# MohaMehrzad/aiOS

Measured on AMD Instinct MI355X. Metric: decode tokens/sec Mistral-7B Q4_K (aggregate over GPUs), higher is better.
Workload: dtype q8_1-act/Q4_K_M; 1 GPU; model=Mistral-7B-Instruct-v0.2 Q4_K_M (architecture: d4096 L32 H32/8 ff14336 V32000), global_batch=1, seq_len=2012, parallelism=dp1, weights=Q4_K_M, per_gpu_batch=1, hipgraph=True

## Files before the change

aios_amd/csrc/bindings.cpp:

```cpp
#include <pybind11/numpy.h>
#include <pybind11/pybind11.h>
#include <pybind11/stl.h>

#include <cstring>

#include "comm.h"
#include "rccl_comm.h"
#include "engine.h"
#include "grammar.h"
#include "ops.h"

namespace py = pybind11;
using namespace aios;

namespace aios {
double bench_launch_chain(int n_kernels, int blocks, int use_graph, int reps);
double bench_stream_read(size_t bytes, int nbuf, int wg_per_cu, int u, int threads, int reps);
double bench_stream_read_part(size_t bytes, int nbuf, int mode, int threads, int reps);
}

namespace {

hipStream_t S(uintptr_t s) { return reinterpret_cast<hipStream_t>(s); }

// ... 427 lines not shown
          a.ts = (unsigned long long*)ts;
          a.block_table = (const int*)block_table; a.bt_rows = bt_rows;
          a.q = (const float*)q; a.k_cache = (const bf16_t*)k; a.v_cache = (const bf16_t*)v;
          a.seq_len = (const int*)seq_len; a.slot = (const int*)slot;
          a.B = B; a.n_heads = H; a.n_kv_heads = Hkv; a.head_dim = hd; a.max_ctx = max_ctx; a.n_chunks = n_chunks;
          a.scale = scale; a.o_part = (float*)opart; a.ml = (float*)ml; a.out = (float*)out;
          a.counters = (int*)counters;
          launch_attn_decode(a, S(st));
        },
        py::arg("q"), py::arg("k"), py::arg("v"), py::arg("seq_len"), py::arg("slot"), py::arg("B"), py::arg("H"),
        py::arg("Hkv"), py::arg("hd"), py::arg("max_ctx"), py::arg("n_chunks"), py::arg("scale"), py::arg("opart"),
        py::arg("ml"), py::arg("out"), py::arg("counters"), py::arg("st"), py::arg("split") = 0,
        py::arg("block_table") = 0, py::arg("bt_rows") = 0, py::arg("ts") = 0, py::arg("kv_fp8") = 0,
        py::arg("k_scale") = 1.f, py::arg("v_scale") = 1.f);
  m.def("attn_decode_split", &attn_decode_split);
  m.def("device_cu_count", [](int dev) {
    int n = 0;
    HIP_CHECK(hipDeviceGetAttribute(&n, hipDeviceAttributeMultiprocessorCount, dev));
    return n;
  }, py::arg("device") = 0);
  m.def("device_pci_bus_id", [](int dev) {
    char buf[64] = {0};
    HIP_CHECK(hipDeviceGetPCIBusId(buf, (int)sizeof(buf), dev));
    return std::string(buf);
  });
  m.def("rmsnorm", [](uintptr_t x, int ldx, uintptr_t w, uintptr_t y, int ldy, int rows, int n, float eps, uintptr_t st) {
    launch_rmsnorm((const float*)x, ldx, (const float*)w, (float*)y, ldy, rows, n, eps, S(st));
  });
  m.def("rmsnorm_bf16", [](uintptr_t x, int ldx, uintptr_t w, uintptr_t y, int ldy, int rows, int n, float eps, uintptr_t st) {
    launch_rmsnorm_bf16((const float*)x, ldx, (const float*)w, (bf16_t*)y, ldy, rows, n, eps, S(st));
// ... 181 lines not shown
```

aios_amd/csrc/engine.hip:

```cpp
#include "engine.h"
#include <hip/hip_ext.h>

#include <set>
#include "comm.h"
#include <cstdlib>
#include <map>

#include <algorithm>
#include <cstring>
#include <cmath>
#include <regex>
#include <sstream>

#include <rocprofiler-sdk-roctx/roctx.h>

namespace aios {

static bool trace_enabled() {
  static const int on = [] {
    const char* e = std::getenv("AIOS_TRACE");
    return e && std::atoi(e) == 0 ? 0 : 1;
  }();
  return on != 0;
}
// ... 42 lines not shown
  if (!cfg_.cu_mask.empty()) {
    int n = 0, dev_cus = 0;
    for (uint32_t w : cfg_.cu_mask) n += __builtin_popcount(w);
    HIP_CHECK(hipDeviceGetAttribute(&dev_cus, hipDeviceAttributeMultiprocessorCount, cfg_.device));
    if (n <= 0) throw std::runtime_error("cu_mask selects no CU");
    HIP_CHECK(hipExtStreamCreateWithCUMask(&stream_, (uint32_t)cfg_.cu_mask.size(), cfg_.cu_mask.data()));
    cus_ = std::min(n, dev_cus);
  } else if (cfg_.stream_priority != 0) {
    int least = 0, greatest = 0;
    HIP_CHECK(hipDeviceGetStreamPriorityRange(&least, &greatest));
    const int pr = std::max(greatest, std::min(least, cfg_.stream_priority));
    HIP_CHECK(hipStreamCreateWithPriority(&stream_, hipStreamNonBlocking, pr));
  } else {
    HIP_CHECK(hipStreamCreateWithFlags(&stream_, hipStreamNonBlocking));
  }

  layers_.resize(cfg_.n_layers);
  if (cfg_.max_batch < 1 || cfg_.max_batch > 64) throw std::runtime_error("max_batch must be 1..64");
  if (cfg_.max_slots < cfg_.max_batch) cfg_.max_slots = cfg_.max_batch;
  if (cfg_.tp_size <= 1 || cfg_.tie_embeddings) cfg_.vocab_parallel = 0;
  if (cfg_.vocab_parallel && cfg_.vocab_size % cfg_.tp_size)
    throw std::runtime_error("vocab_parallel: vocab_size not divisible by tp_size");
}

Engine::~Engine() {
  try {
    stage_release();
  } catch (...) {
  }
  for (auto& kv : graphs_) hipGraphExecDestroy(kv.second);
// ... 1847 lines not shown
```

aios_amd/csrc/gemv.h:

```cpp
#pragma once
#include "common.h"
#include "qweight.h"

namespace aios {

constexpr int GEMV_MAX_SEGS = 3;

enum GemvEpilogue : int {
  EPI_STORE = 0,
  EPI_RESID = 1,
  EPI_SWIGLU = 2,
  EPI_QKV = 3,
  EPI_TP_RESID = 4,
};

struct ArDevCtx;

struct GemvArgs {
  QWeight seg[GEMV_MAX_SEGS];
  int seg_row0[GEMV_MAX_SEGS];
  int nseg;
  int N, K, B;
  int row_base;
  int kt_max;
// ... 22 lines not shown
  const int* pos;
  const int* slot;
  bf16_t* k_cache;
  const int* block_table;
  bf16_t* v_cache;
  int kv_fp8;
  float kv_inv_k, kv_inv_v;
  const int* step_kv;
  const float2* step_rope;
  const ArDevCtx* tp;
  int grid_cap;
  int dry;
};

void launch_gemv(const GemvArgs& a, hipStream_t st);
bool gemv_engine_fits(const GemvArgs& a);
bool gemv_bf16_engine_fits(const GemvArgs& a);
bool launch_gemv_tp_fused(const GemvArgs& a, hipStream_t st);

}
```

aios_amd/csrc/kernels/gemv_cu.h:

```cpp
#pragma once

constexpr int CU_WAVES = 16;
constexpr int CU_THREADS = CU_WAVES * 64;

struct CuPlan {
  int g0;
  int np0;
  int racc_n;
};

template <int CTRL>
__device__ __forceinline__ float cu_dpp(float v) {
  return __int_as_float(__builtin_amdgcn_mov_dpp(__float_as_int(v), CTRL, 0xF, 0xF, false));
}
__device__ __forceinline__ float cu_wave_sum(float v) {
  v += cu_dpp<0xB1>(v);
  v += cu_dpp<0x4E>(v);
  v += cu_dpp<0x141>(v);
  v += cu_dpp<0x140>(v);
  {
    const auto r = __builtin_amdgcn_permlane16_swap(__float_as_uint(v), __float_as_uint(v), false, false);
    v = __uint_as_float(r[0]) + __uint_as_float(r[1]);
  }
  {
// ... 193 lines not shown
  };
  cu_dispatch<DMAX>(min(DMAX, j1 - j0), [&](auto NC) { chunk(NC, std::true_type{}, j0); });
  for (int jb = j0 + DMAX; jb < j1; jb += DMAX)
    cu_dispatch<DMAX>(min(DMAX, j1 - jb), [&](auto NC) { chunk(NC, std::false_type{}, jb); });
  CU_STAMP(4);
}

template <int QT0, int QT1, int D>
__global__ void __launch_bounds__(CU_THREADS) gemv_cu_b1(GemvArgs a, CuPlan pl) {
  static_assert(same_xlayout<QT0, QT1>, "mixed segments must share the activation layout");
  extern __shared__ __attribute__((aligned(16))) float smem[];
  constexpr bool MIXED = QT0 != QT1;
  constexpr int W = QFmt<QT0>::W, R = QFmt<QT0>::RUNS;
  const int nch = a.K / W;
  const int nit = (nch + 63) >> 6;
  const int npairs = a.N >> 1;
  const int lane = threadIdx.x & 63, wave = threadIdx.x >> 6;
  unsigned long long ts[8] = {0, 0, 0, 0, 0, 0, 0, 0};
  CU_STAMP(0);
  auto flush_ts = [&]() {
    if (a.dbg_ts && lane == 0 && (wave == 0 || wave == CU_WAVES - 1))
      for (int i = 0; i < 8; ++i) a.dbg_ts[((size_t)blockIdx.x * 2 + (wave != 0)) * 8 + i] = ts[i];
  };

  const int g = blockIdx.x;
  const bool fmt1 = MIXED && g >= pl.g0;
  int pb, pe;
  if (!fmt1) {
    const int np = MIXED ? pl.np0 : npairs, G = MIXED ? pl.g0 : (int)gridDim.x;
    pb = (int)((long)g * np / G);
    pe = (int)((long)(g + 1) * np / G);
  } else {
    const int np = npairs - pl.np0, G = (int)gridDim.x - pl.g0, gg = g - pl.g0;
    pb = pl.np0 + (int)((long)gg * np / G);
    pe = pl.np0 + (int)((long)(gg + 1) * np / G);
  }
  if (pb >= pe) return;
  const int r0 = 2 * pb, nrows = 2 * (pe - pb);
  const int items = nrows * nit;
  const int ipw = (items + CU_WAVES - 1) / CU_WAVES;
  const int j0 = __builtin_amdgcn_readfirstlane(min(items, wave * ipw));
  const int j1 = __builtin_amdgcn_readfirstlane(min(items, j0 + ipw));

  float* red = smem;
  float* rowacc = smem + 64;
  const int racc_n = pl.racc_n;
  float2* ms = (float2*)(rowacc + racc_n);
  int8_t* xq = (int8_t*)(ms + (size_t)nch * R);
  for (int i = threadIdx.x; i < nrows; i += CU_THREADS) rowacc[i] = 0.f;

  float2 rope = make_float2(1.f, 0.f);
  if (!fmt1) cu_body<QT0, QT0, D>(a, r0, j0, j1, nit, nch, red, rowacc, ms, xq, rope, ts);
  else cu_body<QT1, QT0, D>(a, r0, j0, j1, nit, nch, red, rowacc, ms, xq, rope, ts);
  __syncthreads();
// ... 35 lines not shown
      cu_qkv_epilogue(a, grow, v0, v1, t, pos0, kv_blk0);
    } else {
      gemv_epilogue1(a, grow, v0, v1);
    }
  }
  CU_STAMP(6);
  flush_ts();
}

template <int QT0, int QT1>
inline size_t cu_lds_bytes(const GemvArgs& a, int racc_n) {
  constexpr int W = QFmt<QT0>::W, R = QFmt<QT0>::RUNS;
  return (64 + (size_t)racc_n) * 4 + (size_t)(a.K / W) * R * 8 + (size_t)a.K + 16;
}

inline int cu_fmt_bytes_per_256(int qt) {
  switch (qt) {
    case QT_Q4_K: return 144;
    case QT_Q5_K: return 176;
    case QT_Q6_K: return 210;
    case QT_Q4_0: return 144;
    case QT_Q8_0: return 272;
  }
  return 256;
}

template <int QT0, int QT1>
bool launch_gemv_cu(const GemvArgs& a, hipStream_t st) {
  if constexpr (!same_xlayout<QT0, QT1>) {
    return false;
  } else {
    static const int env = [] {
      const char* e = std::getenv("AIOS_GEMV_CU");
      return e ? std::atoi(e) : 0;
    }();
    const int mode = a.kernel_sel == 2 ? 8 : (a.kernel_sel == 0 ? env : 0);
    if (!mode || a.B != 1 || a.tune_dbg) return false;
    const int npairs = a.N / 2;
    const int cus = device_cu_count();
    const int G = std::min(a.tune_grid > 0 ? a.tune_grid : cus, npairs);
    auto rup = [](int n, int g) { return (n + g - 1) / g; };
    CuPlan pl{G, npairs, (2 * rup(npairs, G) + 3) & ~3};
    if (QT0 != QT1 && a.nseg > 1) {
      const int np0 = a.seg_row0[a.nseg - 1] / 2;
      const double b0 = (double)np0 * cu_fmt_bytes_per_256(QT0), b1 = (double)(npairs - np0) * cu_fmt_bytes_per_256(QT1);
      int g0 = (int)(G * b0 / (b0 + b1) + 0.5);
      g0 = std::max(1, std::min(G - 1, g0));
      if (G < 2 || np0 < 1 || np0 >= npairs) return false;
      const int most = std::max(rup(np0, g0), rup(npairs - np0, G - g0));
      pl = CuPlan{g0, np0, (2 * most + 3) & ~3};
    }
    size_t lds = cu_lds_bytes<QT0, QT1>(a, pl.racc_n);
    if (lds > 160 * 1024) return false;
    lds = std::max(lds, (size_t)(81 * 1024));
    if (mode <= 4)
      hipLaunchKernelGGL((gemv_cu_b1<QT0, QT1, 4>), dim3(G), dim3(CU_THREADS), lds, st, a, pl);
    else
      hipLaunchKernelGGL((gemv_cu_b1<QT0, QT1, 8>), dim3(G), dim3(CU_THREADS), lds, st, a, pl);
    return true;
  }
}
```

aios_amd/csrc/kernels/gemv_dispatch.hip:

```cpp
#include <stdexcept>
#include <string>

#include "../gemv.h"

namespace aios {
void gemv_q4k_q4k(const GemvArgs&, hipStream_t);
void gemv_q4k_q6k(const GemvArgs&, hipStream_t);
void gemv_q6k_q6k(const GemvArgs&, hipStream_t);
void gemv_q5k_q5k(const GemvArgs&, hipStream_t);
void gemv_q5k_q6k(const GemvArgs&, hipStream_t);
void gemv_q4_0(const GemvArgs&, hipStream_t);
void gemv_q8_0(const GemvArgs&, hipStream_t);
void gemv_f16(const GemvArgs&, hipStream_t);
void gemv_bf16(const GemvArgs&, hipStream_t);

bool gemv_q4k_q4k_engine_fits(const GemvArgs&);
bool gemv_q4k_q6k_engine_fits(const GemvArgs&);
bool gemv_q6k_q6k_engine_fits(const GemvArgs&);
bool gemv_q5k_q5k_engine_fits(const GemvArgs&);
bool gemv_q5k_q6k_engine_fits(const GemvArgs&);
bool gemv_q4_0_engine_fits(const GemvArgs&);
bool gemv_q8_0_engine_fits(const GemvArgs&);

bool gemv_engine_fits(const GemvArgs& a) {
// ... 72 lines not shown
```

aios_amd/csrc/kernels/gemv_impl.h:

```cpp
#pragma once
#include <algorithm>

#include "../comm.h"
#include "../common.h"
#include "../gemv.h"
#include "../qweight.h"

namespace aios {

__device__ __forceinline__ QWeight seg_at(const GemvArgs& a, int s) {
  QWeight w;
  w.qtype = s == 0 ? a.seg[0].qtype : (s == 1 ? a.seg[1].qtype : a.seg[2].qtype);
  w.rows = s == 0 ? a.seg[0].rows : (s == 1 ? a.seg[1].rows : a.seg[2].rows);
  w.cols = s == 0 ? a.seg[0].cols : (s == 1 ? a.seg[1].cols : a.seg[2].cols);
  w.pad_ = 0;
  w.p0 = s == 0 ? a.seg[0].p0 : (s == 1 ? a.seg[1].p0 : a.seg[2].p0);
  w.p1 = s == 0 ? a.seg[0].p1 : (s == 1 ? a.seg[1].p1 : a.seg[2].p1);
  w.p2 = s == 0 ? a.seg[0].p2 : (s == 1 ? a.seg[1].p2 : a.seg[2].p2);
  w.p3 = s == 0 ? a.seg[0].p3 : (s == 1 ? a.seg[1].p3 : a.seg[2].p3);
  return w;
}
__device__ __forceinline__ int seg_row0_at(const GemvArgs& a, int s) {
  return s == 0 ? a.seg_row0[0] : (s == 1 ? a.seg_row0[1] : a.seg_row0[2]);
}
// ... 539 lines not shown
```

aios_amd/csrc/kernels/gemv_lds.h:

```cpp
#pragma once

constexpr int LG_NG = 14;
constexpr int LG_NL = 2;
constexpr int LG_THREADS = (LG_NG + LG_NL) * 64;
constexpr int LG_DBG_RING = 0x10000;
#ifndef LG_B0
#define LG_B0 0
#endif

template <int QT>
struct LgPlanes;
template <>
struct LgPlanes<QT_Q4_K> {
  static constexpr int n = 2;
  static constexpr int bpg[4] = {1024, 128, 0, 0};
  static constexpr int dsz[4] = {16, 16, 0, 0};
};
template <>
struct LgPlanes<QT_Q5_K> {
  static constexpr int n = 3;
  static constexpr int bpg[4] = {1024, 128, 256, 0};
  static constexpr int dsz[4] = {16, 16, 16, 0};
};
template <>
// ... 36 lines not shown
}

__device__ __forceinline__ void lg_barrier() {
  asm volatile("" ::: "memory");
  __builtin_amdgcn_s_barrier();
  asm volatile("" ::: "memory");
}

template <int N>
__device__ __forceinline__ void lg_vmcnt() {
  static_assert(N >= 0 && N <= 63, "vmcnt immediate");
  asm volatile("s_waitcnt vmcnt(%0)" ::"n"(N) : "memory");
}

template <int QT>
__device__ __forceinline__ void lg_dma_slot(const GemvArgs& a, uint8_t* dst, int s, int lw, int r0, int nit,
                                            int ngroups) {
  using L = LgLayout<QT>;
  using P = LgPlanes<QT>;
  constexpr int NGS = L::NGS;
  const int lane = threadIdx.x & 63;
  const int g0 = r0 * nit + s * NGS;
  const int glast = r0 * nit + ngroups - 1;
  const int G1 = a.nseg > 1 ? a.seg_row0[1] * nit : 0x7fffffff;
  const int G2 = a.nseg > 2 ? a.seg_row0[2] * nit : 0x7fffffff;
  const int gend = g0 + NGS - 1;
  const int sg0 = g0 >= G2 ? 2 : (g0 >= G1 ? 1 : 0);
  const int Gs = sg0 == 0 ? 0 : (sg0 == 1 ? G1 : G2);
  const int Gn = sg0 == 0 ? G1 : (sg0 == 1 ? G2 : 0x7fffffff);
  const bool fast = gend <= glast && gend < Gn;
  int issued = 0;
  int idx = 0;
  static_for<4>([&](auto pc) {
    constexpr int p = decltype(pc)::value;
    if constexpr (p < P::n) {
      constexpr int S = P::dsz[p], BPG = P::bpg[p];
      constexpr int NI = L::ninst(p);
      const uint8_t* pb0 = sgpr_ptr(lg_plane_ptr(a.seg[0], p));
      const uint8_t* pb1 = sgpr_ptr(lg_plane_ptr(a.seg[1], p));
      const uint8_t* pb2 = sgpr_ptr(lg_plane_ptr(a.seg[2], p));
      if (fast) {
        const __amdgpu_buffer_rsrc_t rs = mk_rsrc(sg0 == 0 ? pb0 : (sg0 == 1 ? pb1 : pb2));
        const int soff0 = (g0 - Gs) * BPG;
#pragma unroll
        for (int i = 0; i < NI; ++i) {
          if ((idx + i) % LG_NL != lw) continue;
          auto* ldst = (__attribute__((address_space(3))) void*)(dst + L::off(p) + i * 64 * S);
          if constexpr (S == 16) __builtin_amdgcn_raw_ptr_buffer_load_lds(rs, ldst, 16, lane * 16, soff0 + i * 1024, 0, 2);
          else __builtin_amdgcn_raw_ptr_buffer_load_lds(rs, ldst, 4, lane * 4, soff0 + i * 256, 0, 2 );
          ++issued;
        }
      } else {
        const uint64_t b0 = (uint64_t)pb0;
        const uint64_t b1 = (uint64_t)pb1 - (uint64_t)(a.nseg > 1 ? G1 : 0) * BPG;
        const uint64_t b2 = (uint64_t)pb2 - (uint64_t)(a.nseg > 2 ? G2 : 0) * BPG;
#pragma unroll
        for (int i = 0; i < NI; ++i) {
          if ((idx + i) % LG_NL != lw) continue;
          const int b = i * 64 * S + lane * S;
          int g = g0 + b / BPG;
          const int o = b & (BPG - 1);
          g = min(g, glast);
          const uint64_t base = g >= G2 ? b2 : (g >= G1 ? b1 : b0);
          const uint8_t* src = (const uint8_t*)(base + (uint64_t)g * BPG + o);
          auto* ldst = (__attribute__((address_space(3))) void*)(dst + L::off(p) + i * 64 * S);
          if constexpr (S == 16) __builtin_amdgcn_global_load_lds((const void*)src, ldst, 16, 0, 2 );
          else __builtin_amdgcn_global_load_lds((const void*)src, ldst, 4, 0, 2 );
          ++issued;
        }
      }
      idx += NI;
    }
  });
  if (issued < L::per_loader) {
    const int g = min(g0, glast);
    const uint64_t b0 = (uint64_t)sgpr_ptr(a.seg[0].p0);
    const uint64_t b1 = (uint64_t)sgpr_ptr(a.seg[1].p0) - (uint64_t)(a.nseg > 1 ? G1 : 0) * 1024;
    const uint64_t b2 = (uint64_t)sgpr_ptr(a.seg[2].p0) - (uint64_t)(a.nseg > 2 ? G2 : 0) * 1024;
    const uint64_t base = g >= G2 ? b2 : (g >= G1 ? b1 : b0);
    const uint8_t* src = (const uint8_t*)(base + (uint64_t)g * 1024 + lane * 16);
    for (; issued < L::per_loader; ++issued)
      __builtin_amdgcn_global_load_lds((const void*)src, (__attribute__((address_space(3))) void*)dst, 16, 0, 2);
  }
}

template <int QT>
__device__ __forceinline__ void lg_read(const uint8_t* slot, int k, int lane, RawChunk& r) {
  using L = LgLayout<QT>;
  const uint8_t* A = slot + L::off(0) + k * 1024;
  r.a = *(const uint4*)(A + lane * 16);
  if constexpr (QT == QT_Q4_K || QT == QT_Q5_K) {
    r.b = *(const uint4*)(slot + L::off(1) + k * 128 + (lane >> 3) * 16);
    if constexpr (QT == QT_Q5_K) r.c = *(const uint4*)(slot + L::off(2) + k * 256 + (lane >> 3) * 32 + 16 * (lane & 1));
  } else if constexpr (QT == QT_Q6_K) {
    const uint2 h = *(const uint2*)(slot + L::off(1) + k * 512 + lane * 8);
    r.b.x = h.x;
    r.b.y = h.y;
    r.c.x = *(const uint16_t*)(slot + L::off(2) + k * 128 + lane * 2);
// ... 113 lines not shown
      if (!valid) m = make_float2(0.f, 0.f);
      acc[b] += sc[rr] * m.x * (float)is[rr] - of[rr] * m.y;
    }
  }
}

template <int QT0, int QT1, int B = 1, int RSUB = 0>
__global__ void __launch_bounds__(LG_THREADS) gemv_lds_b1(GemvArgs a, CuPlan pl) {
  static_assert(same_xlayout<QT0, QT1>, "mixed segments must share the activation layout");
  kernarg_warm<sizeof(GemvArgs) + sizeof(CuPlan)>();
  extern __shared__ __attribute__((aligned(16))) float smem[];
  constexpr bool MIXED = QT0 != QT1;
  constexpr int W = QFmt<QT0>::W, R = QFmt<QT0>::RUNS;
  const int nch = a.K / W;
  const int nit = nch >> 6;
  const int npairs = a.N >> 1;
  const int lane = threadIdx.x & 63;
  const int wave = __builtin_amdgcn_readfirstlane(threadIdx.x >> 6);
  const bool loader = wave >= LG_NG;
  unsigned long long ts[8] = {0, 0, 0, 0, 0, 0, 0, 0};
  CU_STAMP(0);

  const int g = blockIdx.x;
  const bool fmt1 = MIXED && g >= pl.g0;
  int pb, pe;
  if (!fmt1) {
    const int np = MIXED ? pl.np0 : npairs, G = MIXED ? pl.g0 : (int)gridDim.x;
    pb = (int)((long)g * np / G);
    pe = (int)((long)(g + 1) * np / G);
  } else {
    const int np = npairs - pl.np0, G = (int)gridDim.x - pl.g0, gg = g - pl.g0;
    pb = pl.np0 + (int)((long)gg * np / G);
    pe = pl.np0 + (int)((long)(gg + 1) * np / G);
  }
  if (pb >= pe) return;
  const int r0 = 2 * pb, nrows = 2 * (pe - pb);
  const int ngroups = nrows * nit;

  float* red = smem;
  float* rowacc = smem + 64;
  float2* ms = (float2*)(rowacc + B * pl.racc_n);
  int8_t* xq = (int8_t*)(ms + (size_t)B * nch * R);
  const int ring_off = (int)(((const uint8_t*)(xq + (size_t)B * a.K) - (const uint8_t*)smem + 255) & ~255);
  uint8_t* ring = (uint8_t*)smem + ring_off;
  for (int i = threadIdx.x; i < B * pl.racc_n; i += LG_THREADS) rowacc[i] = 0.f;
  if (threadIdx.x < 64) red[threadIdx.x] = 0.f;
  asm volatile("s_waitcnt lgkmcnt(0)" ::: "memory");

  auto loader_path = [&](auto tag) __attribute__((always_inline)) {
    constexpr int QT = decltype(tag)::value;
    using L = LgLayout<QT, RSUB>;
    constexpr int PL = L::per_loader;
    constexpr int LG_R = L::R;
    const int T = (ngroups + L::NGS - 1) / L::NGS;
    const int lw = wave - LG_NG;
    if (LG_B0) lg_barrier();
    const int npro = min(T, LG_R - 1);
    for (int s = 0; s < npro; ++s) lg_dma_slot<QT>(a, ring + (size_t)s * L::slot_bytes, s, lw, r0, nit, ngroups);
    if (npro == LG_R - 1) lg_vmcnt<(LG_R - 2) * PL>();
    else lg_vmcnt<0>();
    lg_barrier();
    for (int t = 0; t < T; ++t) {
      if (t + LG_R - 1 < T) {
        lg_dma_slot<QT>(a, ring + (size_t)((t + LG_R - 1) % LG_R) * L::slot_bytes, t + LG_R - 1, lw, r0, nit,
                        ngroups);
        lg_vmcnt<(LG_R - 2) * PL>();
      } else {
        lg_vmcnt<0>();
      }
      lg_barrier();
    }
    lg_barrier();
  };
  auto consumer_path = [&](auto tag, float2& rope, int& pos0, int& kv_blk0) __attribute__((always_inline)) {
    constexpr int QT = decltype(tag)::value;
    using L = LgLayout<QT, RSUB>;
    constexpr int LG_R = L::R;
    constexpr int GPW = L::GPW;
    const int T = (ngroups + L::NGS - 1) / L::NGS;
    constexpr int NPF = 2;
    StagePre<NPF> pf{};
    q8_stage_prefetch(a, pf, threadIdx.x, LG_NG * 64);
    if (LG_B0) lg_barrier();
    CU_STAMP(1);
    q8_stage<QT0, B, NPF>(a, xq, ms, red, pf, threadIdx.x, LG_NG * 64);
    if (B == 1 && a.epi == EPI_QKV && wave == 0) {
      pos0 = a.pos[0];
      kv_blk0 = kv_block(a.block_table, a.max_ctx / KV_BLOCK, a.slot ? a.slot[0] : 0, pos0);
      if (a.rope_cs) {
        int part, head, lrr;
        qkv_part(a, a.row_base + r0 + 2 * lane, part, head, lrr);
        rope = a.rope_cs[(size_t)pos0 * (a.head_dim >> 1) + (part < 2 ? (lrr >> 1) : 0)];
      }
    }
// ... 203 lines not shown
      }
      lg_barrier();
    }
    CU_STAMP(4);
    asm volatile("s_waitcnt lgkmcnt(0)" ::: "memory");
    lg_barrier();
    CU_STAMP(5);
  };
  float2 rope = make_float2(1.f, 0.f);
  int pos0 = 0, kv_blk0 = 0;
  if (loader) {
    if (!fmt1) loader_path(FmtTag<QT0>{});
    else loader_path(FmtTag<QT1>{});
    return;
  }
  if (!fmt1) consumer_path(FmtTag<QT0>{}, rope, pos0, kv_blk0);
  else consumer_path(FmtTag<QT1>{}, rope, pos0, kv_blk0);
  auto flush_ts = [&]() {
    if (a.dbg_ts && lane == 0 && (wave == 0 || wave == LG_NG - 1))
      for (int i = 0; i < 8; ++i) a.dbg_ts[((size_t)blockIdx.x * 2 + (wave != 0)) * 8 + i] = ts[i];
  };
  if (wave != 0) {
    flush_ts();
    return;
  }

  if constexpr (B > 1) {
    float sb[B];
#pragma unroll
    for (int b = 0; b < B; ++b) {
      sb[b] = 1.f;
      if (a.norm_w) {
        float t = 0.f;
#pragma unroll
        for (int w = 0; w < LG_NG; ++w) t += red[w * B + b];
// ... 69 lines not shown
  } else {
    static const int mode = [] {
      const char* e = std::getenv("AIOS_GEMV_LDS");
      return e ? std::atoi(e) : 1;
    }();
    static const int maxb = [] {
      const char* e = std::getenv("AIOS_GEMV_LDS_MAXB");
      return e ? std::max(1, std::min(4, std::atoi(e))) : 4;
    }();
    if (!mode || a.B < 1 || a.B > (a.kernel_sel == 3 ? 4 : maxb) || (a.tune_dbg & ~LG_DBG_RING) ||
        (a.kernel_sel != 0 && a.kernel_sel != 3))
      return false;
    constexpr int W = QFmt<QT0>::W, R = QFmt<QT0>::RUNS;
    const int nch = a.K / W;
    if (nch % 64) return false;
    const int npairs = a.N / 2;
    const int G = std::min(a.tune_grid > 0 ? a.tune_grid : device_cu_count(), npairs);
    auto rup = [](int n, int g) { return (n + g - 1) / g; };
    CuPlan pl{G, npairs, (2 * rup(npairs, G) + 3) & ~3};
    if (QT0 != QT1 && a.nseg > 1) {
      const int np0 = a.seg_row0[a.nseg - 1] / 2;
      if (G < 2 || np0 < 1 || np0 >= npairs) return false;
      const double b0 = (double)np0 * cu_fmt_bytes_per_256(QT0), b1 = (double)(npairs - np0) * cu_fmt_bytes_per_256(QT1);
      int g0 = (int)(G * b0 / (b0 + b1) + 0.5);
      g0 = std::max(1, std::min(G - 1, g0));
      const int most = std::max(rup(np0, g0), rup(npairs - np0, G - g0));
      pl = CuPlan{g0, np0, (2 * most + 3) & ~3};
    }
    if (mode != 2 && a.kernel_sel != 3 && a.B == 1) {
      static const double min_kb = [] {
        const char* e = std::getenv("AIOS_GEMV_LDS_MIN_KB");
        return e ? std::atof(e) : 40.0;
      }();
      double bytes = 0;
      for (int sg = 0; sg < a.nseg; ++sg)
        bytes += (double)a.seg[sg].rows * a.K / 256.0 * cu_fmt_bytes_per_256(a.seg[sg].qtype);
      if (bytes / G < min_kb * 1024) return false;
    }
    constexpr size_t LDS_MAX = 160 * 1024;
    size_t lds = 0;
    if (a.B == 1) {
      static const int rsub_all = [] {
        const char* e = std::getenv("AIOS_LDS_B1_RSUB");
        return e ? std::atoi(e) : 1;
      }();
      static const int rsub_q6 = [] {
        const char* e = std::getenv("AIOS_LDS_B1_RSUB_Q6");
        return e ? std::atoi(e) : 2;
      }();
      const int rsub = (QT0 == QT_Q6_K && rsub_q6 >= 0) ? rsub_q6 : rsub_all;
      if (rsub == 1 || rsub == 2) {
        if (rsub == 1) lds = lg_lds_bytes<QT0, QT1, 1, 1>(a, pl);
        else lds = lg_lds_bytes<QT0, QT1, 1, 2>(a, pl);
        if (lds > LDS_MAX) return false;
        if (dry) return true;
// ... 36 lines not shown
```

Before: 627.7 tokens/s.

## Precompute per-workgroup GEMV descriptors on host and load via scalar loads

Moves per-workgroup row partitioning and prologue slot classification (fast/seam, segment offset) out of the GEMV kernels into host-built descriptor tables. The tables are cached in device arenas and read with a single 64-byte scalar load. The loader waves issue prologue DMAs straight from these descriptors, and rowacc zeroing moves to the consumer waves only, so the loaders start fetching weights sooner. This adds device-memory descriptors and a mutex-guarded cache with a synchronous upload on first use, which relies on relaxed capture mode to work under graph capture.

New measurement: 640.3 tokens/s (median of 6 runs). 2.0% higher.

```diff
diff --git a/aios_amd/csrc/bindings.cpp b/aios_amd/csrc/bindings.cpp
--- a/aios_amd/csrc/bindings.cpp
+++ b/aios_amd/csrc/bindings.cpp
@@ -7,6 +7,7 @@
 #include "comm.h"
 #include "rccl_comm.h"
 #include "engine.h"
+#include "gemv_desc.h"
 #include "grammar.h"
 #include "ops.h"
 
@@ -465,6 +466,43 @@
         py::arg("block_table") = 0, py::arg("bt_rows") = 0, py::arg("ts") = 0, py::arg("kv_fp8") = 0,
         py::arg("k_scale") = 1.f, py::arg("v_scale") = 1.f);
   m.def("attn_decode_split", &attn_decode_split);
+  m.def("gemv_desc_build",
+        [](std::vector<int> qtypes, std::vector<int> rows, int K, int grid, int variant) -> py::object {
+          if (qtypes.empty() || qtypes.size() > 3 || rows.size() != qtypes.size())
+            throw std::runtime_error("gemv_desc_build: 1..3 segments");
+          GemvDescShape s{};
+          s.nseg = (int)qtypes.size();
+          int r = 0;
+          for (int k = 0; k < s.nseg; ++k) { s.qtype[k] = qtypes[k]; s.seg_row0[k] = r; r += rows[k]; }
+          s.N = r;
+          s.K = K;
+          s.grid = grid;
+          s.variant = variant;
+          CuPlan pl;
+          int G = 0;
+          if (!gemv_desc_plan(s, pl, G)) return py::none();
+          py::list wgs;
+          for (const GemvWgDesc& d : gemv_desc_build(s, pl, G)) {
+            py::dict w;
+            w["r0"] = d.r0; w["nrows"] = d.nrows; w["ngroups"] = d.ngroups; w["T"] = d.T; w["fmt1"] = d.fmt1;
+            w["nfast"] = d.nfast;
+            py::list pro;
+            for (int i = 0; i < GD_PRO; ++i) {
+              py::dict p;
+              p["off"] = d.pro[i] & ((1 << GD_OFF_BITS) - 1);
+              p["seg"] = (d.pro[i] >> GD_SEG_SHIFT) & 3;
+              p["fast"] = (d.pro[i] & GD_FAST) != 0;
+              p["seam"] = (d.pro[i] & GD_SEAM) != 0;
+              pro.append(p);
+            }
+            w["pro"] = pro;
+            wgs.append(w);
+          }
+          py::dict out;
+          out["G"] = G; out["g0"] = pl.g0; out["np0"] = pl.np0; out["racc_n"] = pl.racc_n; out["wgs"] = wgs;
+          return out;
+        },
+        py::arg("qtypes"), py::arg("rows"), py::arg("K"), py::arg("grid"), py::arg("variant") = 3);
   m.def("device_cu_count", [](int dev) {
     int n = 0;
     HIP_CHECK(hipDeviceGetAttribute(&n, hipDeviceAttributeMultiprocessorCount, dev));
diff --git a/aios_amd/csrc/engine.hip b/aios_amd/csrc/engine.hip
--- a/aios_amd/csrc/engine.hip
+++ b/aios_amd/csrc/engine.hip
@@ -80,6 +80,7 @@
   } else {
     HIP_CHECK(hipStreamCreateWithFlags(&stream_, hipStreamNonBlocking));
   }
+  gemv_desc_reserve();
 
   layers_.resize(cfg_.n_layers);
   if (cfg_.max_batch < 1 || cfg_.max_batch > 64) throw std::runtime_error("max_batch must be 1..64");
diff --git a/aios_amd/csrc/gemv.h b/aios_amd/csrc/gemv.h
--- a/aios_amd/csrc/gemv.h
+++ b/aios_amd/csrc/gemv.h
@@ -60,6 +60,7 @@
 };
 
 void launch_gemv(const GemvArgs& a, hipStream_t st);
+void gemv_desc_reserve();
 bool gemv_engine_fits(const GemvArgs& a);
 bool gemv_bf16_engine_fits(const GemvArgs& a);
 bool launch_gemv_tp_fused(const GemvArgs& a, hipStream_t st);
diff --git a/aios_amd/csrc/gemv_desc.h b/aios_amd/csrc/gemv_desc.h
--- /dev/null
+++ b/aios_amd/csrc/gemv_desc.h
@@ -0,0 +1,131 @@
+#pragma once
+#include <algorithm>
+#include <climits>
+#include <vector>
+
+#include "qweight.h"
+
+namespace aios {
+
+struct GemvWgDesc;
+
+struct CuPlan {
+  int g0;
+  int np0;
+  int racc_n;
+  const GemvWgDesc* desc;
+};
+
+constexpr int GD_PRO = 8;
+constexpr int GD_OFF_BITS = 26;
+constexpr int GD_SEG_SHIFT = GD_OFF_BITS;
+constexpr int GD_FAST = 1 << 28;
+constexpr int GD_SEAM = 1 << 29;
+
+struct alignas(64) GemvWgDesc {
+  int r0;
+  int nrows;
+  int ngroups;
+  int T;
+  int fmt1;
+  int nfast;
+  int rsv[2];
+  int pro[GD_PRO];
+};
+static_assert(sizeof(GemvWgDesc) == 64, "one 16-dword scalar load");
+
+struct GemvDescShape {
+  int nseg;
+  int qtype[3];
+  int seg_row0[3];
+  int N, K;
+  int grid;
+  int variant;
+};
+
+inline int gd_chunk_w(int qt) { return qt == QT_Q8_0 ? 16 : ((qt == QT_F16 || qt == QT_BF16) ? 8 : 32); }
+constexpr int gd_slot_groups(int qt) { return (qt == QT_Q6_K || qt == QT_Q5_K) ? 14 : 28; }
+
+inline int cu_fmt_bytes_per_256(int qt) {
+  switch (qt) {
+    case QT_Q4_K: return 144;
+    case QT_Q5_K: return 176;
+    case QT_Q6_K: return 210;
+    case QT_Q4_0: return 144;
+    case QT_Q8_0: return 272;
+  }
+  return 256;
+}
+
+inline bool gemv_desc_plan(const GemvDescShape& s, CuPlan& pl, int& G) {
+  const int npairs = s.N / 2;
+  G = std::min(s.grid, npairs);
+  if (G < 1 || s.nseg < 1 || s.nseg > 3) return false;
+  auto rup = [](int n, int g) { return (n + g - 1) / g; };
+  pl = CuPlan{G, npairs, (2 * rup(npairs, G) + 3) & ~3, nullptr};
+  const int qt0 = s.qtype[0], qt1 = s.qtype[s.nseg - 1];
+  if (qt0 != qt1 && s.nseg > 1) {
+    const int np0 = s.seg_row0[s.nseg - 1] / 2;
+    if (G < 2 || np0 < 1 || np0 >= npairs) return false;
+    const double b0 = (double)np0 * cu_fmt_bytes_per_256(qt0), b1 = (double)(npairs - np0) * cu_fmt_bytes_per_256(qt1);
+    int g0 = (int)(G * b0 / (b0 + b1) + 0.5);
+    g0 = std::max(1, std::min(G - 1, g0));
+    const int most = std::max(rup(np0, g0), rup(npairs - np0, G - g0));
+    pl = CuPlan{g0, np0, (2 * most + 3) & ~3, nullptr};
+  }
+  return true;
+}
+
+inline std::vector<GemvWgDesc> gemv_desc_build(const GemvDescShape& s, const CuPlan& pl, int G) {
+  std::vector<GemvWgDesc> out((size_t)G);
+  const int qt0 = s.qtype[0], qt1 = s.qtype[s.nseg - 1];
+  const bool mixed = qt0 != qt1;
+  const int npairs = s.N / 2;
+  const int nch = s.K / gd_chunk_w(qt0);
+  const int nit = (nch + 63) >> 6;
+  const long G1 = s.nseg > 1 ? (long)s.seg_row0[1] * nit : LONG_MAX;
+  const long G2 = s.nseg > 2 ? (long)s.seg_row0[2] * nit : LONG_MAX;
+  for (int g = 0; g < G; ++g) {
+    GemvWgDesc d{};
+    const bool fmt1 = mixed && g >= pl.g0;
+    int pb, pe;
+    if (!fmt1) {
+      const int np = mixed ? pl.np0 : npairs, Gd = mixed ? pl.g0 : G;
+      pb = (int)((long)g * np / Gd);
+      pe = (int)((long)(g + 1) * np / Gd);
+    } else {
+      const int np = npairs - pl.np0, Gd = G - pl.g0, gg = g - pl.g0;
+      pb = pl.np0 + (int)((long)gg * np / Gd);
+      pe = pl.np0 + (int)((long)(gg + 1) * np / Gd);
+    }
+    d.fmt1 = fmt1;
+    if (pb < pe) {
+      d.r0 = 2 * pb;
+      d.nrows = 2 * (pe - pb);
+      d.ngroups = d.nrows * nit;
+      const int ngs = gd_slot_groups(fmt1 ? qt1 : qt0);
+      d.T = (d.ngroups + ngs - 1) / ngs;
+      const long gfirst = (long)d.r0 * nit, glast = gfirst + d.ngroups - 1;
+      bool lead = true;
+      for (int sl = 0; sl < std::min(d.T, GD_PRO); ++sl) {
+        const long g0 = gfirst + (long)sl * ngs, gend = g0 + ngs - 1;
+        const int sg = g0 >= G2 ? 2 : (g0 >= G1 ? 1 : 0);
+        const long Gs = sg == 0 ? 0 : (sg == 1 ? G1 : G2), Gn = sg == 0 ? G1 : (sg == 1 ? G2 : LONG_MAX);
+        const long off = g0 - Gs;
+        const bool whole = gend <= glast && off < (1L << GD_OFF_BITS);
+        const bool fast = whole && gend < Gn;
+        d.pro[sl] = (int)(off & ((1L << GD_OFF_BITS) - 1)) | (sg << GD_SEG_SHIFT) | (fast ? GD_FAST : 0) |
+                    (whole && !fast ? GD_SEAM : 0);
+        lead = lead && fast;
+        if (lead) d.nfast = sl + 1;
+      }
+    }
+    out[(size_t)g] = d;
+  }
+  return out;
+}
+
+const GemvWgDesc* gemv_desc_device(const GemvDescShape& s, const CuPlan& pl, int G);
+void gemv_desc_reserve();
+
+}
diff --git a/aios_amd/csrc/kernels/gemv_cu.h b/aios_amd/csrc/kernels/gemv_cu.h
--- a/aios_amd/csrc/kernels/gemv_cu.h
+++ b/aios_amd/csrc/kernels/gemv_cu.h
@@ -3,11 +3,32 @@
 constexpr int CU_WAVES = 16;
 constexpr int CU_THREADS = CU_WAVES * 64;
 
-struct CuPlan {
-  int g0;
-  int np0;
-  int racc_n;
-};
+
+__device__ __forceinline__ GemvWgDesc gd_load(const GemvWgDesc* base) {
+  typedef int v16i __attribute__((ext_vector_type(16)));
+  using cp_t = const __attribute__((address_space(4))) v16i*;
+  const v16i v = *((cp_t)(uintptr_t)base + blockIdx.x);
+  GemvWgDesc d;
+  d.r0 = v[0]; d.nrows = v[1]; d.ngroups = v[2]; d.T = v[3]; d.fmt1 = v[4]; d.nfast = v[5];
+  d.rsv[0] = d.rsv[1] = 0;
+#pragma unroll
+  for (int i = 0; i < GD_PRO; ++i) d.pro[i] = v[8 + i];
+  return d;
+}
+
+inline GemvDescShape cu_desc_shape(const GemvArgs& a, int grid, int variant) {
+  GemvDescShape s{};
+  s.nseg = a.nseg;
+  for (int k = 0; k < a.nseg; ++k) {
+    s.qtype[k] = a.seg[k].qtype;
+    s.seg_row0[k] = a.seg_row0[k];
+  }
+  s.N = a.N;
+  s.K = a.K;
+  s.grid = grid;
+  s.variant = variant;
+  return s;
+}
 
 template <int CTRL>
 __device__ __forceinline__ float cu_dpp(float v) {
@@ -231,7 +252,6 @@
   constexpr int W = QFmt<QT0>::W, R = QFmt<QT0>::RUNS;
   const int nch = a.K / W;
   const int nit = (nch + 63) >> 6;
-  const int npairs = a.N >> 1;
   const int lane = threadIdx.x & 63, wave = threadIdx.x >> 6;
   unsigned long long ts[8] = {0, 0, 0, 0, 0, 0, 0, 0};
   CU_STAMP(0);
@@ -240,21 +260,11 @@
       for (int i = 0; i < 8; ++i) a.dbg_ts[((size_t)blockIdx.x * 2 + (wave != 0)) * 8 + i] = ts[i];
   };
 
-  const int g = blockIdx.x;
-  const bool fmt1 = MIXED && g >= pl.g0;
-  int pb, pe;
-  if (!fmt1) {
-    const int np = MIXED ? pl.np0 : npairs, G = MIXED ? pl.g0 : (int)gridDim.x;
-    pb = (int)((long)g * np / G);
-    pe = (int)((long)(g + 1) * np / G);
-  } else {
-    const int np = npairs - pl.np0, G = (int)gridDim.x - pl.g0, gg = g - pl.g0;
-    pb = pl.np0 + (int)((long)gg * np / G);
-    pe = pl.np0 + (int)((long)(gg + 1) * np / G);
-  }
-  if (pb >= pe) return;
-  const int r0 = 2 * pb, nrows = 2 * (pe - pb);
-  const int items = nrows * nit;
+  const GemvWgDesc d = gd_load(pl.desc);
+  if (d.nrows == 0) return;
+  const bool fmt1 = MIXED && d.fmt1;
+  const int r0 = d.r0, nrows = d.nrows;
+  const int items = d.ngroups;
   const int ipw = (items + CU_WAVES - 1) / CU_WAVES;
   const int j0 = __builtin_amdgcn_readfirstlane(min(items, wave * ipw));
   const int j1 = __builtin_amdgcn_readfirstlane(min(items, j0 + ipw));
@@ -320,17 +330,6 @@
   return (64 + (size_t)racc_n) * 4 + (size_t)(a.K / W) * R * 8 + (size_t)a.K + 16;
 }
 
-inline int cu_fmt_bytes_per_256(int qt) {
-  switch (qt) {
-    case QT_Q4_K: return 144;
-    case QT_Q5_K: return 176;
-    case QT_Q6_K: return 210;
-    case QT_Q4_0: return 144;
-    case QT_Q8_0: return 272;
-  }
-  return 256;
-}
-
 template <int QT0, int QT1>
 bool launch_gemv_cu(const GemvArgs& a, hipStream_t st) {
   if constexpr (!same_xlayout<QT0, QT1>) {
@@ -342,23 +341,14 @@
     }();
     const int mode = a.kernel_sel == 2 ? 8 : (a.kernel_sel == 0 ? env : 0);
     if (!mode || a.B != 1 || a.tune_dbg) return false;
-    const int npairs = a.N / 2;
-    const int cus = device_cu_count();
-    const int G = std::min(a.tune_grid > 0 ? a.tune_grid : cus, npairs);
-    auto rup = [](int n, int g) { return (n + g - 1) / g; };
-    CuPlan pl{G, npairs, (2 * rup(npairs, G) + 3) & ~3};
-    if (QT0 != QT1 && a.nseg > 1) {
-      const int np0 = a.seg_row0[a.nseg - 1] / 2;
-      const double b0 = (double)np0 * cu_fmt_bytes_per_256(QT0), b1 = (double)(npairs - np0) * cu_fmt_bytes_per_256(QT1);
-      int g0 = (int)(G * b0 / (b0 + b1) + 0.5);
-      g0 = std::max(1, std::min(G - 1, g0));
-      if (G < 2 || np0 < 1 || np0 >= npairs) return false;
-      const int most = std::max(rup(np0, g0), rup(npairs - np0, G - g0));
-      pl = CuPlan{g0, np0, (2 * most + 3) & ~3};
-    }
+    const GemvDescShape sh = cu_desc_shape(a, a.tune_grid > 0 ? a.tune_grid : device_cu_count(), 2);
+    CuPlan pl;
+    int G;
+    if (!gemv_desc_plan(sh, pl, G)) return false;
     size_t lds = cu_lds_bytes<QT0, QT1>(a, pl.racc_n);
     if (lds > 160 * 1024) return false;
     lds = std::max(lds, (size_t)(81 * 1024));
+    pl.desc = gemv_desc_device(sh, pl, G);
     if (mode <= 4)
       hipLaunchKernelGGL((gemv_cu_b1<QT0, QT1, 4>), dim3(G), dim3(CU_THREADS), lds, st, a, pl);
     else
diff --git a/aios_amd/csrc/kernels/gemv_dispatch.hip b/aios_amd/csrc/kernels/gemv_dispatch.hip
--- a/aios_amd/csrc/kernels/gemv_dispatch.hip
+++ b/aios_amd/csrc/kernels/gemv_dispatch.hip
@@ -1,9 +1,79 @@
+#include <array>
+#include <map>
+#include <mutex>
 #include <stdexcept>
 #include <string>
 
 #include "../gemv.h"
+#include "../gemv_desc.h"
 
 namespace aios {
+
+namespace {
+struct DescArena {
+  GemvWgDesc* dev = nullptr;
+  size_t cap = 0, used = 0;
+};
+struct DescDevice {
+  std::vector<DescArena> arenas;
+  hipStream_t st = nullptr;
+  std::map<std::array<int, 14>, const GemvWgDesc*> cache;
+};
+std::mutex g_desc_mu;
+std::map<int, DescDevice> g_desc_dev;
+constexpr size_t DESC_ARENA_RECORDS = 32768;
+
+struct RelaxedCapture {
+  hipStreamCaptureMode mode = hipStreamCaptureModeRelaxed;
+  RelaxedCapture() { (void)hipThreadExchangeStreamCaptureMode(&mode); }
+  ~RelaxedCapture() { (void)hipThreadExchangeStreamCaptureMode(&mode); }
+};
+
+GemvWgDesc* desc_alloc(DescDevice& d, size_t n) {
+  if (d.arenas.empty() || d.arenas.back().used + n > d.arenas.back().cap) {
+    DescArena a;
+    a.cap = std::max(n, DESC_ARENA_RECORDS);
+    HIP_CHECK(hipMalloc((void**)&a.dev, a.cap * sizeof(GemvWgDesc)));
+    d.arenas.push_back(a);
+  }
+  DescArena& a = d.arenas.back();
+  GemvWgDesc* p = a.dev + a.used;
+  a.used += n;
+  return p;
+}
+}
+
+void gemv_desc_reserve() {
+  int dev = 0;
+  HIP_CHECK(hipGetDevice(&dev));
+  std::lock_guard<std::mutex> lk(g_desc_mu);
+  DescDevice& d = g_desc_dev[dev];
+  RelaxedCapture rc;
+  if (!d.st) HIP_CHECK(hipStreamCreateWithFlags(&d.st, hipStreamNonBlocking));
+  if (d.arenas.empty()) {
+    desc_alloc(d, 1);
+    d.arenas.back().used = 0;
+  }
+}
+
+const GemvWgDesc* gemv_desc_device(const GemvDescShape& s, const CuPlan& pl, int G) {
+  int dev = 0;
+  HIP_CHECK(hipGetDevice(&dev));
+  const std::array<int, 14> key = {s.nseg, s.qtype[0], s.qtype[1], s.qtype[2], s.seg_row0[0], s.seg_row0[1],
+                                   s.seg_row0[2], s.N, s.K, s.grid, s.variant, G, pl.g0, pl.np0};
+  std::lock_guard<std::mutex> lk(g_desc_mu);
+  DescDevice& d = g_desc_dev[dev];
+  auto it = d.cache.find(key);
+  if (it != d.cache.end()) return it->second;
+  const std::vector<GemvWgDesc> host = gemv_desc_build(s, pl, G);
+  RelaxedCapture rc;
+  if (!d.st) HIP_CHECK(hipStreamCreateWithFlags(&d.st, hipStreamNonBlocking));
+  GemvWgDesc* p = desc_alloc(d, host.size());
+  HIP_CHECK(hipMemcpyAsync(p, host.data(), host.size() * sizeof(GemvWgDesc), hipMemcpyHostToDevice, d.st));
+  HIP_CHECK(hipStreamSynchronize(d.st));
+  d.cache.emplace(key, p);
+  return p;
+}
 void gemv_q4k_q4k(const GemvArgs&, hipStream_t);
 void gemv_q4k_q6k(const GemvArgs&, hipStream_t);
 void gemv_q6k_q6k(const GemvArgs&, hipStream_t);
diff --git a/aios_amd/csrc/kernels/gemv_impl.h b/aios_amd/csrc/kernels/gemv_impl.h
--- a/aios_amd/csrc/kernels/gemv_impl.h
+++ b/aios_amd/csrc/kernels/gemv_impl.h
@@ -4,6 +4,7 @@
 #include "../comm.h"
 #include "../common.h"
 #include "../gemv.h"
+#include "../gemv_desc.h"
 #include "../qweight.h"
 
 namespace aios {
diff --git a/aios_amd/csrc/kernels/gemv_lds.h b/aios_amd/csrc/kernels/gemv_lds.h
--- a/aios_amd/csrc/kernels/gemv_lds.h
+++ b/aios_amd/csrc/kernels/gemv_lds.h
@@ -74,21 +74,10 @@
 }
 
 template <int QT>
-__device__ __forceinline__ void lg_dma_slot(const GemvArgs& a, uint8_t* dst, int s, int lw, int r0, int nit,
-                                            int ngroups) {
+__device__ __forceinline__ void lg_dma_fast(const GemvArgs& a, uint8_t* dst, int seg, int goff, int lw) {
   using L = LgLayout<QT>;
   using P = LgPlanes<QT>;
-  constexpr int NGS = L::NGS;
   const int lane = threadIdx.x & 63;
-  const int g0 = r0 * nit + s * NGS;
-  const int glast = r0 * nit + ngroups - 1;
-  const int G1 = a.nseg > 1 ? a.seg_row0[1] * nit : 0x7fffffff;
-  const int G2 = a.nseg > 2 ? a.seg_row0[2] * nit : 0x7fffffff;
-  const int gend = g0 + NGS - 1;
-  const int sg0 = g0 >= G2 ? 2 : (g0 >= G1 ? 1 : 0);
-  const int Gs = sg0 == 0 ? 0 : (sg0 == 1 ? G1 : G2);
-  const int Gn = sg0 == 0 ? G1 : (sg0 == 1 ? G2 : 0x7fffffff);
-  const bool fast = gend <= glast && gend < Gn;
   int issued = 0;
   int idx = 0;
   static_for<4>([&](auto pc) {
@@ -99,35 +88,56 @@
       const uint8_t* pb0 = sgpr_ptr(lg_plane_ptr(a.seg[0], p));
       const uint8_t* pb1 = sgpr_ptr(lg_plane_ptr(a.seg[1], p));
       const uint8_t* pb2 = sgpr_ptr(lg_plane_ptr(a.seg[2], p));
-      if (fast) {
-        const __amdgpu_buffer_rsrc_t rs = mk_rsrc(sg0 == 0 ? pb0 : (sg0 == 1 ? pb1 : pb2));
-        const int soff0 = (g0 - Gs) * BPG;
-#pragma unroll
-        for (int i = 0; i < NI; ++i) {
-          if ((idx + i) % LG_NL != lw) continue;
-          auto* ldst = (__attribute__((address_space(3))) void*)(dst + L::off(p) + i * 64 * S);
-          if constexpr (S == 16) __builtin_amdgcn_raw_ptr_buffer_load_lds(rs, ldst, 16, lane * 16, soff0 + i * 1024, 0, 2);
-          else __builtin_amdgcn_raw_ptr_buffer_load_lds(rs, ldst, 4, lane * 4, soff0 + i * 256, 0, 2 );
-          ++issued;
-        }
-      } else {
-        const uint64_t b0 = (uint64_t)pb0;
-        const uint64_t b1 = (uint64_t)pb1 - (uint64_t)(a.nseg > 1 ? G1 : 0) * BPG;
-        const uint64_t b2 = (uint64_t)pb2 - (uint64_t)(a.nseg > 2 ? G2 : 0) * BPG;
-#pragma unroll
-        for (int i = 0; i < NI; ++i) {
-          if ((idx + i) % LG_NL != lw) continue;
-          const int b = i * 64 * S + lane * S;
-          int g = g0 + b / BPG;
-          const int o = b & (BPG - 1);
-          g = min(g, glast);
-          const uint64_t base = g >= G2 ? b2 : (g >= G1 ? b1 : b0);
-          const uint8_t* src = (const uint8_t*)(base + (uint64_t)g * BPG + o);
-          auto* ldst = (__attribute__((address_space(3))) void*)(dst + L::off(p) + i * 64 * S);
-          if constexpr (S == 16) __builtin_amdgcn_global_load_lds((const void*)src, ldst, 16, 0, 2 );
-          else __builtin_amdgcn_global_load_lds((const void*)src, ldst, 4, 0, 2 );
-          ++issued;
-        }
+      const __amdgpu_buffer_rsrc_t rs = mk_rsrc(seg == 0 ? pb0 : (seg == 1 ? pb1 : pb2));
+      const int soff0 = goff * BPG;
+#pragma unroll
+      for (int i = 0; i < NI; ++i) {
+        if ((idx + i) % LG_NL != lw) continue;
+        auto* ldst = (__attribute__((address_space(3))) void*)(dst + L::off(p) + i * 64 * S);
+        if constexpr (S == 16) __builtin_amdgcn_raw_ptr_buffer_load_lds(rs, ldst, 16, lane * 16, soff0 + i * 1024, 0, 2);
+        else __builtin_amdgcn_raw_ptr_buffer_load_lds(rs, ldst, 4, lane * 4, soff0 + i * 256, 0, 2 );
+        ++issued;
+      }
+      if constexpr (p == 0) {
+        if ((L::total_inst % LG_NL) != 0 && lw >= L::total_inst % LG_NL)
+          __builtin_amdgcn_raw_ptr_buffer_load_lds(rs, (__attribute__((address_space(3))) void*)dst, 16, lane * 16, soff0,
+                                                   0, 2);
+      }
+      idx += NI;
+    }
+  });
+  (void)issued;
+}
+
+template <int QT>
+__device__ __forceinline__ void lg_dma_general(const GemvArgs& a, uint8_t* dst, int g0, int glast, int G1, int G2,
+                                               int lw) {
+  using L = LgLayout<QT>;
+  using P = LgPlanes<QT>;
+  const int lane = threadIdx.x & 63;
+  int issued = 0;
+  int idx = 0;
+  static_for<4>([&](auto pc) {
+    constexpr int p = decltype(pc)::value;
+    if constexpr (p < P::n) {
+      constexpr int S = P::dsz[p], BPG = P::bpg[p];
+      constexpr int NI = L::ninst(p);
+      const uint64_t b0 = (uint64_t)sgpr_ptr(lg_plane_ptr(a.seg[0], p));
+      const uint64_t b1 = (uint64_t)sgpr_ptr(lg_plane_ptr(a.seg[1], p)) - (uint64_t)(a.nseg > 1 ? G1 : 0) * BPG;
+      const uint64_t b2 = (uint64_t)sgpr_ptr(lg_plane_ptr(a.seg[2], p)) - (uint64_t)(a.nseg > 2 ? G2 : 0) * BPG;
+#pragma unroll
+      for (int i = 0; i < NI; ++i) {
+        if ((idx + i) % LG_NL != lw) continue;
+        const int b = i * 64 * S + lane * S;
+        int g = g0 + b / BPG;
+        const int o = b & (BPG - 1);
+        g = min(g, glast);
+        const uint64_t base = g >= G2 ? b2 : (g >= G1 ? b1 : b0);
+        const uint8_t* src = (const uint8_t*)(base + (uint64_t)g * BPG + o);
+        auto* ldst = (__attribute__((address_space(3))) void*)(dst + L::off(p) + i * 64 * S);
+        if constexpr (S == 16) __builtin_amdgcn_global_load_lds((const void*)src, ldst, 16, 0, 2 );
+        else __builtin_amdgcn_global_load_lds((const void*)src, ldst, 4, 0, 2 );
+        ++issued;
       }
       idx += NI;
     }
@@ -142,6 +152,22 @@
     for (; issued < L::per_loader; ++issued)
       __builtin_amdgcn_global_load_lds((const void*)src, (__attribute__((address_space(3))) void*)dst, 16, 0, 2);
   }
+}
+
+template <int QT>
+__device__ __forceinline__ void lg_dma_slot(const GemvArgs& a, uint8_t* dst, int s, int lw, int r0, int nit,
+                                            int ngroups) {
+  constexpr int NGS = LgLayout<QT>::NGS;
+  const int g0 = r0 * nit + s * NGS;
+  const int glast = r0 * nit + ngroups - 1;
+  const int G1 = a.nseg > 1 ? a.seg_row0[1] * nit : 0x7fffffff;
+  const int G2 = a.nseg > 2 ? a.seg_row0[2] * nit : 0x7fffffff;
+  const int gend = g0 + NGS - 1;
+  const int sg0 = g0 >= G2 ? 2 : (g0 >= G1 ? 1 : 0);
+  const int Gs = sg0 == 0 ? 0 : (sg0 == 1 ? G1 : G2);
+  const int Gn = sg0 == 0 ? G1 : (sg0 == 1 ? G2 : 0x7fffffff);
+  if (gend <= glast && gend < Gn) lg_dma_fast<QT>(a, dst, sg0, g0 - Gs, lw);
+  else lg_dma_general<QT>(a, dst, g0, glast, G1, G2, lw);
 }
 
 template <int QT>
@@ -285,28 +311,17 @@
   constexpr int W = QFmt<QT0>::W, R = QFmt<QT0>::RUNS;
   const int nch = a.K / W;
   const int nit = nch >> 6;
-  const int npairs = a.N >> 1;
   const int lane = threadIdx.x & 63;
   const int wave = __builtin_amdgcn_readfirstlane(threadIdx.x >> 6);
   const bool loader = wave >= LG_NG;
   unsigned long long ts[8] = {0, 0, 0, 0, 0, 0, 0, 0};
   CU_STAMP(0);
 
-  const int g = blockIdx.x;
-  const bool fmt1 = MIXED && g >= pl.g0;
-  int pb, pe;
-  if (!fmt1) {
-    const int np = MIXED ? pl.np0 : npairs, G = MIXED ? pl.g0 : (int)gridDim.x;
-    pb = (int)((long)g * np / G);
-    pe = (int)((long)(g + 1) * np / G);
-  } else {
-    const int np = npairs - pl.np0, G = (int)gridDim.x - pl.g0, gg = g - pl.g0;
-    pb = pl.np0 + (int)((long)gg * np / G);
-    pe = pl.np0 + (int)((long)(gg + 1) * np / G);
-  }
-  if (pb >= pe) return;
-  const int r0 = 2 * pb, nrows = 2 * (pe - pb);
-  const int ngroups = nrows * nit;
+  const GemvWgDesc d = gd_load(pl.desc);
+  if (d.nrows == 0) return;
+  const bool fmt1 = MIXED && d.fmt1;
+  const int r0 = d.r0, nrows = d.nrows;
+  const int ngroups = d.ngroups;
 
   float* red = smem;
   float* rowacc = smem + 64;
@@ -314,20 +329,34 @@
   int8_t* xq = (int8_t*)(ms + (size_t)B * nch * R);
   const int ring_off = (int)(((const uint8_t*)(xq + (size_t)B * a.K) - (const uint8_t*)smem + 255) & ~255);
   uint8_t* ring = (uint8_t*)smem + ring_off;
-  for (int i = threadIdx.x; i < B * pl.racc_n; i += LG_THREADS) rowacc[i] = 0.f;
-  if (threadIdx.x < 64) red[threadIdx.x] = 0.f;
-  asm volatile("s_waitcnt lgkmcnt(0)" ::: "memory");
 
   auto loader_path = [&](auto tag) __attribute__((always_inline)) {
     constexpr int QT = decltype(tag)::value;
     using L = LgLayout<QT, RSUB>;
     constexpr int PL = L::per_loader;
     constexpr int LG_R = L::R;
-    const int T = (ngroups + L::NGS - 1) / L::NGS;
+    static_assert(L::NGS == gd_slot_groups(QT), "the descriptor's slot count assumes this slot size");
+    static_assert(LG_R - 1 <= GD_PRO, "prologue slots described per workgroup");
+    const int T = d.T;
     const int lw = wave - LG_NG;
     if (LG_B0) lg_barrier();
     const int npro = min(T, LG_R - 1);
-    for (int s = 0; s < npro; ++s) lg_dma_slot<QT>(a, ring + (size_t)s * L::slot_bytes, s, lw, r0, nit, ngroups);
+    if (d.nfast >= npro) {
+      static_for<LG_R - 1>([&](auto sc) {
+        constexpr int s = decltype(sc)::value;
+        if (s < npro) {
+          lg_dma_fast<QT>(a, ring + (size_t)s * L::slot_bytes, (d.pro[s] >> GD_SEG_SHIFT) & 3,
+                          d.pro[s] & ((1 << GD_OFF_BITS) - 1), lw);
+          if constexpr (s == 0) CU_STAMP(1);
+        }
+      });
+    } else {
+      for (int s = 0; s < npro; ++s) {
+        lg_dma_slot<QT>(a, ring + (size_t)s * L::slot_bytes, s, lw, r0, nit, ngroups);
+        if (s == 0) CU_STAMP(1);
+      }
+    }
+    CU_STAMP(2);
     if (npro == LG_R - 1) lg_vmcnt<(LG_R - 2) * PL>();
     else lg_vmcnt<0>();
     lg_barrier();
@@ -342,13 +371,18 @@
       lg_barrier();
     }
     lg_barrier();
+    if (AIOS_GEMV_PROBES && a.dbg_ts && lane == 0 && lw == 0) {
+      a.dbg_ts[((size_t)blockIdx.x * 2 + 0) * 8 + 7] = ts[0];
+      a.dbg_ts[((size_t)blockIdx.x * 2 + 1) * 8 + 6] = ts[1];
+      a.dbg_ts[((size_t)blockIdx.x * 2 + 1) * 8 + 7] = ts[2];
+    }
   };
   auto consumer_path = [&](auto tag, float2& rope, int& pos0, int& kv_blk0) __attribute__((always_inline)) {
     constexpr int QT = decltype(tag)::value;
     using L = LgLayout<QT, RSUB>;
     constexpr int LG_R = L::R;
     constexpr int GPW = L::GPW;
-    const int T = (ngroups + L::NGS - 1) / L::NGS;
+    const int T = d.T;
     constexpr int NPF = 2;
     StagePre<NPF> pf{};
     q8_stage_prefetch(a, pf, threadIdx.x, LG_NG * 64);
@@ -582,11 +616,14 @@
     else loader_path(FmtTag<QT1>{});
     return;
   }
+  for (int i = threadIdx.x; i < B * pl.racc_n; i += LG_NG * 64) rowacc[i] = 0.f;
+  if (threadIdx.x < 64) red[threadIdx.x] = 0.f;
+  asm volatile("s_waitcnt lgkmcnt(0)" ::: "memory");
   if (!fmt1) consumer_path(FmtTag<QT0>{}, rope, pos0, kv_blk0);
   else consumer_path(FmtTag<QT1>{}, rope, pos0, kv_blk0);
   auto flush_ts = [&]() {
     if (a.dbg_ts && lane == 0 && (wave == 0 || wave == LG_NG - 1))
-      for (int i = 0; i < 8; ++i) a.dbg_ts[((size_t)blockIdx.x * 2 + (wave != 0)) * 8 + i] = ts[i];
+      for (int i = 0; i < (wave != 0 ? 6 : 7); ++i) a.dbg_ts[((size_t)blockIdx.x * 2 + (wave != 0)) * 8 + i] = ts[i];
   };
   if (wave != 0) {
     flush_ts();
@@ -686,19 +723,10 @@
     constexpr int W = QFmt<QT0>::W, R = QFmt<QT0>::RUNS;
     const int nch = a.K / W;
     if (nch % 64) return false;
-    const int npairs = a.N / 2;
-    const int G = std::min(a.tune_grid > 0 ? a.tune_grid : device_cu_count(), npairs);
-    auto rup = [](int n, int g) { return (n + g - 1) / g; };
-    CuPlan pl{G, npairs, (2 * rup(npairs, G) + 3) & ~3};
-    if (QT0 != QT1 && a.nseg > 1) {
-      const int np0 = a.seg_row0[a.nseg - 1] / 2;
-      if (G < 2 || np0 < 1 || np0 >= npairs) return false;
-      const double b0 = (double)np0 * cu_fmt_bytes_per_256(QT0), b1 = (double)(npairs - np0) * cu_fmt_bytes_per_256(QT1);
-      int g0 = (int)(G * b0 / (b0 + b1) + 0.5);
-      g0 = std::max(1, std::min(G - 1, g0));
-      const int most = std::max(rup(np0, g0), rup(npairs - np0, G - g0));
-      pl = CuPlan{g0, np0, (2 * most + 3) & ~3};
-    }
+    const GemvDescShape sh = cu_desc_shape(a, a.tune_grid > 0 ? a.tune_grid : device_cu_count(), 3);
+    CuPlan pl;
+    int G;
+    if (!gemv_desc_plan(sh, pl, G)) return false;
     if (mode != 2 && a.kernel_sel != 3 && a.B == 1) {
       static const double min_kb = [] {
         const char* e = std::getenv("AIOS_GEMV_LDS_MIN_KB");
@@ -711,6 +739,7 @@
     }
     constexpr size_t LDS_MAX = 160 * 1024;
     size_t lds = 0;
+    if (!dry) pl.desc = gemv_desc_device(sh, pl, G);
     if (a.B == 1) {
       static const int rsub_all = [] {
         const char* e = std::getenv("AIOS_LDS_B1_RSUB");
```
